# rohitsinghlab/SAME

Measured on AMD Instinct MI355X. Metric: cell-pairs/sec on 100k×100k cost build + edge-cross sweep; % HBM roofline, higher is better.
Workload: dtype f64

## Files before the change

### same_amd/csrc/delaunay_dev.hip

```cpp
#include "qhull_margin.h"
#include "window_internal.h"

namespace {

using namespace devmath;
using namespace win;
using scan::Pair;

constexpr int NB_CAP = 128;
constexpr int OWN_CAP = 32;
constexpr int SURV_CAP = 1024;
constexpr int SCAN_CELLS_CAP = 256;
constexpr double SIGN_MARGIN = 1e-12;
constexpr double SCREEN_SLACK = 1e-9;

enum { ST_STATUS = 0, ST_TRIS = 1, ST_WORDS = 8 };

struct Par {
    double x0, y0, cw, r2s, delta, w, sc_m;
    qm::Scale sc;
    double ox[8], oy[8];
    int nx, ny, ncell, n_oct;
};

struct Job {
    const double *xy;
    int64_t n, ncell_cap, cap_out;
    unsigned long long *st;
    unsigned long long *scan_cells, *scan_own;
    unsigned *cell_cnt, *cell_start, *slot, *own_cnt;
    int32_t *cell_of, *sorted, *own_tris, *out;
    Par *par;
};

struct Settings {
    double radius, cos_thr, guard;
};

__device__ __forceinline__ void refuse(const Job &j, unsigned bits) { atomicOr(&j.st[ST_STATUS], (unsigned long long)bits); }
__device__ __forceinline__ unsigned long long status_of(const Job &j) {
    return __hip_atomic_load(&j.st[ST_STATUS], __ATOMIC_RELAXED, __HIP_MEMORY_SCOPE_AGENT);
}
__device__ __forceinline__ int cell_x(const Par &p, double x) {
    const double f = std::floor((x - p.x0) / p.cw);
    return !(f >= 0.0) ? 0 : (f >= (double)p.nx ? p.nx - 1 : (int)f);
}
__device__ __forceinline__ int cell_y(const Par &p, double y) {
    const double f = std::floor((y - p.y0) / p.cw);
    return !(f >= 0.0) ? 0 : (f >= (double)p.ny ? p.ny - 1 : (int)f);
}

__device__ __forceinline__ double block_min(double v, double *sh) {
#pragma unroll
    for (int off = 32; off > 0; off >>= 1) v = fmin(v, __shfl_xor(v, off, 64));
    __syncthreads();
    if ((threadIdx.x & 63) == 0) sh[threadIdx.x >> 6] = v;
    __syncthreads();
    return fmin(fmin(sh[0], sh[1]), fmin(sh[2], sh[3]));
}
__device__ __forceinline__ void block_argmax(double &v, int64_t &i, double *shv, int64_t *shi) {
#pragma unroll
    for (int off = 32; off > 0; off >>= 1) {
        const double ov = __shfl_xor(v, off, 64);
        const int64_t oi = __shfl_xor(i, off, 64);
        if (ov > v || (ov == v && oi < i)) { v = ov; i = oi; }
    }
    __syncthreads();
    if ((threadIdx.x & 63) == 0) { shv[threadIdx.x >> 6] = v; shi[threadIdx.x >> 6] = i; }
    __syncthreads();
    v = shv[0];
    i = shi[0];
    for (int q = 1; q < 4; ++q)
        if (shv[q] > v || (shv[q] == v && shi[q] < i)) { v = shv[q]; i = shi[q]; }
}

__device__ __forceinline__ double oct_dir(int k, double x, double y) {
    switch (k) {
        case 0: return -y;
        case 1: return x - y;
        case 2: return x;
        case 3: return x + y;
        case 4: return y;
        case 5: return y - x;
        case 6: return -x;
        default: return -x - y;
    }
}

__global__ __launch_bounds__(256) void dd_setup_kernel(Batch<Job> b, Settings set) {
    const Job &j = b.w[blockIdx.y];
    __shared__ double shv[4];
    __shared__ int64_t shi[4];
    const int64_t n = j.n;
    double mnx = __builtin_inf(), mny = mnx, mxx = mnx, mxy = mnx, zmin = mnx, zmax = mnx, m = mnx;
    bool bad = false;
    double ov[8];
    int64_t oi[8];
    for (int k = 0; k < 8; ++k) { ov[k] = -__builtin_inf(); oi[k] = INT64_MAX; }
    for (int64_t i = threadIdx.x; i < n; i += blockDim.x) {
        const double x = j.xy[2 * i], y = j.xy[2 * i + 1];
        if (!(std::isfinite(x) && std::isfinite(y))) { bad = true; continue; }
        const double z = x * x + y * y;
        mnx = fmin(mnx, x); mxx = fmin(mxx, -x); mny = fmin(mny, y); mxy = fmin(mxy, -y);
        zmin = fmin(zmin, z); zmax = fmin(zmax, -z);
        m = fmin(m, -fmax(std::fabs(x), std::fabs(y)));
        for (int k = 0; k < 8; ++k) {
            const double v = oct_dir(k, x, y);
            if (v > ov[k] || (v == ov[k] && i < oi[k])) { ov[k] = v; oi[k] = i; }
        }
    }
    if (bad) refuse(j, SAME_DD_NONFINITE);
    mnx = block_min(mnx, shv); mxx = -block_min(mxx, shv); mny = block_min(mny, shv); mxy = -block_min(mxy, shv);
    zmin = block_min(zmin, shv); zmax = -block_min(zmax, shv); m = -block_min(m, shv);
    for (int k = 0; k < 8; ++k) block_argmax(ov[k], oi[k], shv, shi);
    if (threadIdx.x != 0) return;
    Par &p = *j.par;
    if (n < 3) { refuse(j, SAME_DD_FEW_POINTS); p.nx = p.ny = p.ncell = 1; p.n_oct = 0; p.x0 = p.y0 = 0.0; p.cw = 1.0; return; }
    p.sc = qm::scale(m, zmin, zmax);
    const double w = fmax(mxx - mnx, mxy - mny);
    p.w = w;
    p.sc_m = m;
    p.x0 = mnx;
    p.y0 = mny;
    p.r2s = (set.radius * (1.0 + SCREEN_SLACK)) * (set.radius * (1.0 + SCREEN_SLACK));
    double cw = set.radius * (1.0 + 1e-6);
    int64_t nx = 1, ny = 1;
    for (int it = 0; it < 64; ++it) {
        const double fx = std::floor((mxx - mnx) / cw) + 1.0, fy = std::floor((mxy - mny) / cw) + 1.0;
        if (fx * fy <= (double)j.ncell_cap) { nx = (int64_t)fx; ny = (int64_t)fy; break; }
        cw *= 2.0;
        nx = 0;
    }
    if (nx == 0 || !(cw > 0.0) || !std::isfinite(cw)) { refuse(j, SAME_DD_OVERFLOW); nx = ny = 1; }
    p.cw = cw;
    p.nx = (int)nx;
    p.ny = (int)ny;
    p.ncell = (int)(nx * ny);
    p.delta = 4.0 * set.guard * p.sc.allow + 64.0 * qm::EPS * (w + m);
    int c = 0;
    for (int k = 0; k < 8; ++k) {
        const int64_t i = oi[k];
        if (i < 0 || i >= n) continue;
        const double x = j.xy[2 * i], y = j.xy[2 * i + 1];
        if (c > 0 && x == p.ox[c - 1] && y == p.oy[c - 1]) continue;
        if (k == 7 && c > 0 && x == p.ox[0] && y == p.oy[0]) continue;
        p.ox[c] = x;
        p.oy[c] = y;
        ++c;
    }
    p.n_oct = c;
}

__global__ __launch_bounds__(256) void dd_count_kernel(Batch<Job> b) {
    const Job &j = b.w[blockIdx.y];
    const int64_t i = (int64_t)blockIdx.x * blockDim.x + threadIdx.x;
    if (i >= j.n || j.n < 3) return;
    const Par &p = *j.par;
    const int c = cell_y(p, j.xy[2 * i + 1]) * p.nx + cell_x(p, j.xy[2 * i]);
    j.cell_of[i] = c;
    j.slot[i] = atomicAdd(&j.cell_cnt[c], 1u);
}
__global__ __launch_bounds__(scan::NT) void dd_cell_scan_kernel(Batch<Job> b) {
    __shared__ scan::Shared sh;
    const Job &j = b.w[blockIdx.y];
    if (j.n < 3) return;
    const int64_t nc = j.par->ncell;
    const int nb = (int)scan::blocks_for(nc);
    if ((int)blockIdx.x >= nb) return;
    const unsigned *cnt = j.cell_cnt;
    auto val = [&](int64_t c) { return Pair{c < nc ? cnt[c] : 0u, 0u}; };
    Pair through;
    const Pair off = scan::exclusive(j.scan_cells, (int)blockIdx.x, val, sh, &through);
    const int64_t c = (int64_t)blockIdx.x * scan::NT + threadIdx.x;
    if (c < nc) j.cell_start[c] = off.a;
    if ((int)blockIdx.x == nb - 1 && threadIdx.x == 0) j.cell_start[nc] = through.a;
}
__global__ __launch_bounds__(256) void dd_scatter_kernel(Batch<Job> b) {
    const Job &j = b.w[blockIdx.y];
    const int64_t i = (int64_t)blockIdx.x * blockDim.x + threadIdx.x;
    if (i >= j.n || j.n < 3) return;
    const int64_t at = (int64_t)j.cell_start[j.cell_of[i]] + j.slot[i];
    if (at >= 0 && at < j.n) j.sorted[at] = (int32_t)i;
}
__global__ __launch_bounds__(256) void dd_cell_sort_kernel(Batch<Job> b) {
    const Job &j = b.w[blockIdx.y];
    const int64_t c = (int64_t)blockIdx.x * blockDim.x + threadIdx.x;
    if (j.n < 3 || c >= j.par->ncell) return;
    const int64_t lo = j.cell_start[c], hi = j.cell_start[c + 1];
    if (lo < 0 || hi > j.n) return;
    int32_t *s = j.sorted;
    for (int64_t a = lo + 1; a < hi; ++a) {
        const int32_t v = s[a];
        int64_t q = a - 1;
        while (q >= lo && s[q] > v) { s[q + 1] = s[q]; --q; }
        s[q + 1] = v;
    }
}

__device__ __forceinline__ double cross3(double ax, double ay, double bx, double by, double cx, double cy) {
    return (bx - ax) * (cy - ay) - (by - ay) * (cx - ax);
}

__global__ __launch_bounds__(256) void dd_hull_kernel(Batch<Job> b, Settings set) {
    const Job &j = b.w[blockIdx.y];
    if (j.n < 3 || status_of(j)) return;
    const Par &p = *j.par;
    __shared__ double ux[SURV_CAP], uy[SURV_CAP], sx[SURV_CAP], sy[SURV_CAP];
    __shared__ int32_t ui[SURV_CAP], si[SURV_CAP];
    __shared__ int hull[2 * SURV_CAP + 2];
    __shared__ int n_surv, n_hull, verdict;
    if (threadIdx.x == 0) { n_surv = 0; n_hull = 0; verdict = 0; }
    __syncthreads();
    const int n_oct = p.n_oct;
    for (int64_t i = threadIdx.x; i < j.n; i += blockDim.x) {
        const double x = j.xy[2 * i], y = j.xy[2 * i + 1];
        bool deep = n_oct >= 3;
        for (int k = 0; k < n_oct && deep; ++k) {
            const int k1 = k + 1 == n_oct ? 0 : k + 1;
            const double ex = p.ox[k1] - p.ox[k], ey = p.oy[k1] - p.oy[k];
            const double len = std::sqrt(ex * ex + ey * ey);
            deep = cross3(p.ox[k], p.oy[k], p.ox[k1], p.oy[k1], x, y) > p.delta * len + 16.0 * qm::EPS * (p.sc_m + p.w) * (len + 2.0 * p.w);
        }
        if (!deep) {
            const int at = atomicAdd(&n_surv, 1);
            if (at < SURV_CAP) { ux[at] = x; uy[at] = y; ui[at] = (int32_t)i; }
        }
    }
    __syncthreads();
    const int k = n_surv;
    if (k > SURV_CAP || k < 3) {
        if (threadIdx.x == 0) refuse(j, k > SURV_CAP ? SAME_DD_OVERFLOW : SAME_DD_IN_DOUBT);
        return;
    }
    for (int a = threadIdx.x; a < k; a += blockDim.x) {
        int r = 0;
        for (int c = 0; c < k; ++c)
            r += ux[c] < ux[a] || (ux[c] == ux[a] && (uy[c] < uy[a] || (uy[c] == uy[a] && ui[c] < ui[a])));
        sx[r] = ux[a]; sy[r] = uy[a]; si[r] = ui[a];
    }
    __syncthreads();
    if (threadIdx.x == 0) {
        int h = 0;
        for (int a = 0; a < k; ++a) {
            while (h >= 2 && cross3(sx[hull[h - 2]], sy[hull[h - 2]], sx[hull[h - 1]], sy[hull[h - 1]], sx[a], sy[a]) <= 0.0) --h;
            hull[h++] = a;
        }
        for (int a = k - 2, lo = h + 1; a >= 0; --a) {
            while (h >= lo && cross3(sx[hull[h - 2]], sy[hull[h - 2]], sx[hull[h - 1]], sy[hull[h - 1]], sx[a], sy[a]) <= 0.0) --h;
            hull[h++] = a;
        }
        n_hull = h - 1;
        if (n_hull < 3) verdict = 1;
    }
    __syncthreads();
    const int h = n_hull;
    if (!verdict) {
        for (int t = threadIdx.x; t < h; t += blockDim.x) {
            const int a = hull[(t + h - 1) % h], c = hull[t], d = hull[(t + 1) % h];
            const double area2 = std::fabs(cross3(sx[a], sy[a], sx[c], sy[c], sx[d], sy[d]));
            const double chord = std::sqrt((sx[d] - sx[a]) * (sx[d] - sx[a]) + (sy[d] - sy[a]) * (sy[d] - sy[a]));
            if (!(qm::plain_ratio(area2, chord, p.sc) > set.guard)) atomicOr(&verdict, 1);
        }
        for (int64_t q = threadIdx.x; q < (int64_t)k * h; q += blockDim.x) {
            const int s = (int)(q / h), e = (int)(q % h);
            const int a = hull[e], c = hull[(e + 1) % h];
            if (s == a || s == c) continue;
            const double area2 = std::fabs(cross3(sx[a], sy[a], sx[c], sy[c], sx[s], sy[s]));
            const double edge = std::sqrt((sx[c] - sx[a]) * (sx[c] - sx[a]) + (sy[c] - sy[a]) * (sy[c] - sy[a]));
            if (!(qm::plain_ratio(area2, edge, p.sc) > set.guard)) atomicOr(&verdict, 1);
        }
    }
    __syncthreads();
    if (threadIdx.x == 0 && verdict) refuse(j, SAME_DD_IN_DOUBT);
}

__device__ __forceinline__ double max_corner_cos(double2_t a, double2_t b, double2_t c) {
    const double c1 = corner_cos(b, a, c), c2 = corner_cos(a, b, c), c3 = corner_cos(a, c, b);
    return fmax(fmax(c1, c2), c3);
}

__global__ __launch_bounds__(256) void dd_candidate_kernel(Batch<Job> b, Settings set) {
    const Job &j = b.w[blockIdx.y];
    const int64_t pi = (int64_t)blockIdx.x * blockDim.x + threadIdx.x;
    if (pi >= j.n || j.n < 3 || status_of(j)) return;
    const Par &p = *j.par;
    const double *__restrict__ xy = j.xy;
    const int32_t *__restrict__ sorted = j.sorted;
    const unsigned *__restrict__ start = j.cell_start;
    const double2_t P = ld2(xy, pi);
    const int c0 = j.cell_of[pi], cx = c0 % p.nx, cy = c0 / p.nx;
    int32_t nb[NB_CAP];
    int k = 0;
    for (int yy = cy - 1; yy <= cy + 1; ++yy) {
        if (yy < 0 || yy >= p.ny) continue;
        for (int xx = cx - 1; xx <= cx + 1; ++xx) {
            if (xx < 0 || xx >= p.nx) continue;
            const int c = yy * p.nx + xx;
            for (unsigned q = start[c]; q < start[c + 1]; ++q) {
                const int32_t s = sorted[q];
                if (s <= pi) continue;
                const double2_t S = ld2(xy, s);
                const double dx = S.x - P.x, dy = S.y - P.y;
                if (dx * dx + dy * dy >= p.r2s) continue;
                if (k == NB_CAP) { refuse(j, SAME_DD_OVERFLOW); return; }
                nb[k++] = s;
            }
        }
    }
    for (int a = 1; a < k; ++a) {
        const int32_t v = nb[a];
        int q = a - 1;
        while (q >= 0 && nb[q] > v) { nb[q + 1] = nb[q]; --q; }
        nb[q + 1] = v;
    }
    int32_t *own = j.own_tris + pi * (int64_t)OWN_CAP * 3;
    unsigned count = 0;
    for (int a = 0; a < k; ++a) {
        const double2_t Q = ld2(xy, nb[a]);
        for (int bq = a + 1; bq < k; ++bq) {
            const double2_t R = ld2(xy, nb[bq]);
            const double qx = R.x - Q.x, qy = R.y - Q.y;
            if (qx * qx + qy * qy >= p.r2s) continue;
            if (!(max_corner_cos(P, Q, R) < set.cos_thr + SCREEN_SLACK)) continue;
            double2_t B = Q, C = R;
            int32_t ib = nb[a], ic = nb[bq];
            const double o = cross3(P.x, P.y, Q.x, Q.y, R.x, R.y);
            if (o < 0.0) { B = R; C = Q; ib = nb[bq]; ic = nb[a]; }
            const double dx = B.x - P.x, dy = B.y - P.y, ex = C.x - P.x, ey = C.y - P.y;
            const double bl = dx * dx + dy * dy, cl = ex * ex + ey * ey, d = dx * ey - dy * ex;
            if (!(d > 0.0)) { refuse(j, SAME_DD_IN_DOUBT); return; }
            const double ucx = (ey * bl - dy * cl) * 0.5 / d, ucy = (dx * cl - ex * bl) * 0.5 / d;
            const double ccx = P.x + ucx, ccy = P.y + ucy, rad = std::sqrt(ucx * ucx + ucy * ucy);
            const double jd = qm::judge(P.x, P.y, dx, dy, ex, ey, p.sc);
            const double reach = 2.0 * set.guard / (rad * d * jd) + 1e-9 * rad + 1e-12 * (std::fabs(ccx) + std::fabs(ccy));
            const int x_lo = cell_x(p, ccx - (rad + reach)), x_hi = cell_x(p, ccx + (rad + reach));
            const int y_lo = cell_y(p, ccy - (rad + reach)), y_hi = cell_y(p, ccy + (rad + reach));
            if (!(reach < 1e300) || (int64_t)(x_hi - x_lo + 1) * (y_hi - y_lo + 1) > SCAN_CELLS_CAP) { refuse(j, SAME_DD_OVERFLOW); return; }
            bool inside = false, doubt = false;
            for (int yy = y_lo; yy <= y_hi && !inside; ++yy) {
                for (int xx = x_lo; xx <= x_hi && !inside; ++xx) {
                    const int c = yy * p.nx + xx;
                    for (unsigned q = start[c]; q < start[c + 1]; ++q) {
                        const int32_t s = sorted[q];
                        if (s == pi || s == ib || s == ic) continue;
                        const double2_t S = ld2(xy, s);
                        const double ax_ = P.x - S.x, ay_ = P.y - S.y, bx_ = B.x - S.x, by_ = B.y - S.y, fx = C.x - S.x, fy = C.y - S.y;
                        const double ap = ax_ * ax_ + ay_ * ay_, bp = bx_ * bx_ + by_ * by_, cp = fx * fx + fy * fy;
                        const double det = ax_ * (by_ * cp - bp * fy) - ay_ * (bx_ * cp - bp * fx) + ap * (bx_ * fy - by_ * fx);
                        const double perm = (std::fabs(by_ * cp) + std::fabs(bp * fy)) * std::fabs(ax_) +
                                            (std::fabs(bx_ * cp) + std::fabs(bp * fx)) * std::fabs(ay_) +
                                            (std::fabs(bx_ * fy) + std::fabs(by_ * fx)) * ap;
                        if (!(std::fabs(det) > SIGN_MARGIN * perm) || !(std::fabs(det) * jd > set.guard)) {
                            doubt = true;
                            continue;
                        }
                        if (det > 0.0) { inside = true; break; }
                    }
                }
            }
            if (inside) continue;
            if (doubt) { refuse(j, SAME_DD_IN_DOUBT); return; }
            if (count == OWN_CAP) { refuse(j, SAME_DD_OVERFLOW); return; }
            own[3 * count] = (int32_t)pi;
            own[3 * count + 1] = ib;
            own[3 * count + 2] = ic;
            ++count;
        }
    }
    j.own_cnt[pi] = count;
}

__global__ __launch_bounds__(scan::NT) void dd_emit_kernel(Batch<Job> b) {
    __shared__ scan::Shared sh;
    const Job &j = b.w[blockIdx.y];
    if (j.n < 3) return;
    const int64_t n = j.n;
    const int nb = (int)scan::blocks_for(n);
    if ((int)blockIdx.x >= nb) return;
    const unsigned *cnt = j.own_cnt;
    auto val = [&](int64_t i) { return Pair{i < n ? cnt[i] : 0u, 0u}; };
    Pair through;
    const Pair off = scan::exclusive(j.scan_own, (int)blockIdx.x, val, sh, &through);
    const int64_t i = (int64_t)blockIdx.x * scan::NT + threadIdx.x;
    if (i < n) {
        const unsigned c = cnt[i];
        if (c > (unsigned)OWN_CAP || (int64_t)off.a + c > j.cap_out) {
            refuse(j, SAME_DD_OVERFLOW);
        } else {
            const int32_t *src = j.own_tris + i * (int64_t)OWN_CAP * 3;
            int32_t *dst = j.out + 3 * (int64_t)off.a;
            for (unsigned q = 0; q < 3 * c; ++q) dst[q] = src[q];
        }
    }
    if ((int)blockIdx.x == nb - 1 && threadIdx.x == 0) j.st[ST_TRIS] = through.a;
}

struct Layout {
    size_t o_st, o_scan_cells, o_cell_cnt, o_own_cnt, o_scan_own, zero_bytes, o_par, o_cell_start, o_cell_of, o_slot, o_sorted, o_own, total;
    int64_t ncell_cap;
};
Layout layout_for(int64_t n) {
    Layout l{};
    l.ncell_cap = 2 * n + 64;
    Carver cv;
    l.o_st = cv.take(ST_WORDS * 8);
    l.o_scan_cells = cv.take(scan::status_bytes(l.ncell_cap));
    l.o_cell_cnt = cv.take((size_t)l.ncell_cap * 4);
    l.o_own_cnt = cv.take((size_t)n * 4);
    l.o_scan_own = cv.take(scan::status_bytes(n));
    l.zero_bytes = cv.off;
    l.o_par = cv.take(sizeof(Par));
    l.o_cell_start = cv.take((size_t)(l.ncell_cap + 1) * 4);
    l.o_cell_of = cv.take((size_t)n * 4);
    l.o_slot = cv.take((size_t)n * 4);
    l.o_sorted = cv.take((size_t)n * 4);
    l.o_own = cv.take((size_t)n * OWN_CAP * 12);
    l.total = cv.off;
    return l;
}
Job job_on(char *base, const Layout &l, const double *xy, int64_t n, int32_t *out, int64_t cap_out) {
    Job j{};
    j.xy = xy;
    j.n = n;
    j.ncell_cap = l.ncell_cap;
    j.cap_out = cap_out;
    j.st = reinterpret_cast<unsigned long long *>(base + l.o_st);
    j.scan_cells = scan::arg(reinterpret_cast<unsigned long long *>(base + l.o_scan_cells));
    j.cell_cnt = reinterpret_cast<unsigned *>(base + l.o_cell_cnt);
    j.own_cnt = reinterpret_cast<unsigned *>(base + l.o_own_cnt);
    j.scan_own = scan::arg(reinterpret_cast<unsigned long long *>(base + l.o_scan_own));
    j.par = reinterpret_cast<Par *>(base + l.o_par);
    j.cell_start = reinterpret_cast<unsigned *>(base + l.o_cell_start);
    j.cell_of = reinterpret_cast<int32_t *>(base + l.o_cell_of);
    j.slot = reinterpret_cast<unsigned *>(base + l.o_slot);
    j.sorted = reinterpret_cast<int32_t *>(base + l.o_sorted);
    j.own_tris = reinterpret_cast<int32_t *>(base + l.o_own);
    j.out = out;
    return j;
}

int launch_group(same_ctx *ctx, const Job *jobs, int n_j, Settings set) {
    Batch<Job> b{};
    int64_t max_n = 0, max_cells = 0;
    for (int q = 0; q < n_j; ++q) {
        b.w[q] = jobs[q];
        max_n = std::max(max_n, jobs[q].n);
        max_cells = std::max(max_cells, jobs[q].ncell_cap);
    }
    const unsigned nw = (unsigned)n_j;
    SAME_LAUNCH(ctx, dd_setup_kernel, dim3(1, nw), dim3(256), 0, b, set);
    SAME_LAUNCH(ctx, dd_count_kernel, dim3(grid_for(max_n), nw), dim3(256), 0, b);
    SAME_LAUNCH(ctx, dd_cell_scan_kernel, dim3(scan::blocks_for(max_cells), nw), dim3(scan::NT), 0, b);
    SAME_LAUNCH(ctx, dd_scatter_kernel, dim3(grid_for(max_n), nw), dim3(256), 0, b);
    SAME_LAUNCH(ctx, dd_cell_sort_kernel, dim3(grid_for(max_cells), nw), dim3(256), 0, b);
    SAME_LAUNCH(ctx, dd_hull_kernel, dim3(1, nw), dim3(256), 0, b, set);
    SAME_LAUNCH(ctx, dd_candidate_kernel, dim3(grid_for(max_n), nw), dim3(256), 0, b, set);
    SAME_LAUNCH(ctx, dd_emit_kernel, dim3(scan::blocks_for(max_n), nw), dim3(scan::NT), 0, b);
    HIP_TRY(ctx, hipGetLastError());
    return SAME_OK;
}

bool settings_answerable(double radius, int angle_enabled, double cos_thr) {
    return radius > 0.0 && std::isfinite(radius) && angle_enabled && cos_thr == cos_thr && cos_thr < 0.9999;
}

}

extern "C" {

int same_window_delaunay(same_window *const *windows, int n_windows, double radius, int angle_enabled, double cos_thr, double guard,
                         int32_t *out_status, int64_t *out_n_tris) {
    same_ctx *ctx = nullptr;
    SAME_TRY(check_batch(windows, n_windows, &ctx));
    REQUIRE(ctx, out_status && out_n_tris && guard >= 0.0);
    for (int i = 0; i < n_windows; ++i) REQUIRE(ctx, windows[i]->staged == 2 && windows[i]->n_ua < ((int64_t)1 << 30));
    SAME_TRY(same_use(ctx));
    const bool ok = settings_answerable(radius, angle_enabled, cos_thr);
    const Settings set{radius, cos_thr, guard};
    std::vector<Job> jobs;
    std::vector<int> at((size_t)n_windows, -1);
    for (int i = 0; i < n_windows; ++i) {
        same_window *w = windows[i];
        w->dd_ok = 0;
        w->n_dd = 0;
        out_status[i] = !ok ? SAME_DD_NO_ANGLE : (w->n_ua < 3 ? SAME_DD_FEW_POINTS : 0);
        out_n_tris[i] = 0;
        if (out_status[i]) continue;
        const int64_t n = w->n_ua, cap_out = 2 * n;
        const Layout l = layout_for(n);
        SAME_TRY(ensure(ctx, w->dd_work, l.total));
        SAME_TRY(ensure(ctx, w->dd_tris, (size_t)cap_out * 12));
        at[(size_t)i] = (int)jobs.size();
        jobs.push_back(job_on(static_cast<char *>(w->dd_work.p), l, w->axy_c, n, static_cast<int32_t *>(w->dd_tris.p), cap_out));
        jobs.back().ncell_cap = l.ncell_cap;
    }
    if (jobs.empty()) return SAME_OK;
    int rc = SAME_OK;
    for (size_t g = 0; g < jobs.size() && rc == SAME_OK; g += SAME_LAUNCH_WINDOWS) {
        const int n_g = (int)std::min<size_t>(SAME_LAUNCH_WINDOWS, jobs.size() - g);
        ZeroArgs zr[SAME_LAUNCH_WINDOWS];
        for (int q = 0; q < n_g; ++q) {
            const Job &jb = jobs[g + (size_t)q];
            zr[q] = ZeroArgs{{jb.st, nullptr}, {layout_for(jb.n).zero_bytes, 0}};
        }
        rc = launch_zero(ctx, zr, n_g);
        if (rc == SAME_OK) rc = launch_group(ctx, jobs.data() + g, n_g, set);
    }
    unsigned long long *h = static_cast<unsigned long long *>(ctx->pinned);
    for (size_t q = 0; q < jobs.size() && rc == SAME_OK; ++q) {
        hipError_t e = hipMemcpyAsync(h + 2 * q, jobs[q].st, 16, hipMemcpyDeviceToHost, ctx->stream);
        ++ctx->stats[SAME_STAT_COPIES];
        if (e != hipSuccess) rc = same_fail(ctx, SAME_EIO, "device triangulation status", e);
    }
    if (rc != SAME_OK) {
        (void)hipStreamSynchronize(ctx->stream);
        return rc;
    }
    SAME_WAIT(ctx);
    for (int i = 0; i < n_windows; ++i) {
        if (at[(size_t)i] < 0) continue;
        const unsigned long long *s = h + 2 * at[(size_t)i];
        same_window *w = windows[i];
        out_status[i] = (int32_t)(s[0] & 0x7fffffffu);
        if (out_status[i] == 0) {
            w->n_dd = (int64_t)s[1];
            w->dd_ok = 1;
            out_n_tris[i] = w->n_dd;
        }
    }
    return SAME_OK;
}

int same_delaunay_filtered(same_ctx *ctx, const double *xy, int64_t n, double radius, int angle_enabled, double cos_thr, double guard,
                           int32_t *out_tris, int64_t cap, int64_t *out_n_tris, int32_t *out_status) {
    if (!ctx) return SAME_EINVAL;
    REQUIRE(ctx, (xy || n == 0) && out_n_tris && out_status && n >= 0 && n < ((int64_t)1 << 30) && cap >= 0 && (out_tris || cap == 0) &&
                     guard >= 0.0);
    *out_n_tris = 0;
    *out_status = !settings_answerable(radius, angle_enabled, cos_thr) ? SAME_DD_NO_ANGLE : (n < 3 ? SAME_DD_FEW_POINTS : 0);
    if (*out_status) return SAME_OK;
    SAME_TRY(same_use(ctx));
    const Layout l = layout_for(n);
    double *dxy = nullptr;
    char *work = nullptr;
    int32_t *dout = nullptr;
    SAME_TRY(up_as(ctx, SL_AXY, xy, (size_t)n * 2, &dxy));
    SAME_TRY(slot_as(ctx, SL_X, l.total, &work));
    SAME_TRY(slot_as(ctx, SL_TRIS, (size_t)(2 * n) * 3, &dout));
    Job jb = job_on(work, l, dxy, n, dout, 2 * n);
    SAME_FILL(ctx, work, 0, l.zero_bytes);
    SAME_TRY(launch_group(ctx, &jb, 1, Settings{radius, cos_thr, guard}));
    unsigned long long *h = static_cast<unsigned long long *>(ctx->pinned);
    SAME_COPY(ctx, h, jb.st, 16, hipMemcpyDeviceToHost);
    SAME_WAIT(ctx);
    *out_status = (int32_t)(h[0] & 0x7fffffffu);
    if (*out_status) return SAME_OK;
    const int64_t count = (int64_t)h[1];
    if (count > cap) return SAME_EINVAL;
    if (count) {
        SAME_COPY(ctx, out_tris, dout, (size_t)count * 12, hipMemcpyDeviceToHost);
        SAME_WAIT(ctx);
    }
    *out_n_tris = count;
    return SAME_OK;
}

}
```

Baseline: 634.9 billion.

## Restructure Delaunay candidate kernel into wave-per-point with shared-memory cell staging

Replaces the one-thread-per-point candidate kernel with a cell-strided grid where each block stages a 5x5 cell neighbourhood of points into LDS. Each wavefront handles one owner point and distributes neighbour gathering, candidate triangle setup and in-circle tests across its lanes using ballots. The aim is to remove divergent serial loops and repeated global gathers of point coordinates. It adds LDS pressure, extra syncs and counters, and a global fallback path when the stage overflows or a circle reaches beyond the staged area.

```diff
diff --git a/same_amd/csrc/delaunay_dev.hip b/same_amd/csrc/delaunay_dev.hip
--- a/same_amd/csrc/delaunay_dev.hip
+++ b/same_amd/csrc/delaunay_dev.hip
@@ -14,7 +14,7 @@
 constexpr double SIGN_MARGIN = 1e-12;
 constexpr double SCREEN_SLACK = 1e-9;
 
-enum { ST_STATUS = 0, ST_TRIS = 1, ST_WORDS = 8 };
+enum { ST_STATUS = 0, ST_TRIS = 1, ST_FAR = 2, ST_UNSTAGED = 3, ST_WORDS = 8 };
 
 struct Par {
     double x0, y0, cw, r2s, delta, w, sc_m;
@@ -278,96 +278,304 @@
     const double c1 = corner_cos(b, a, c), c2 = corner_cos(a, b, c), c3 = corner_cos(a, c, b);
     return fmax(fmax(c1, c2), c3);
 }
-
-__global__ __launch_bounds__(256) void dd_candidate_kernel(Batch<Job> b, Settings set) {
+__device__ __forceinline__ bool near_owner(const Par &p, double2_t P, double2_t S) {
+    const double dx = S.x - P.x, dy = S.y - P.y;
+    return !(dx * dx + dy * dy >= p.r2s);
+}
+__device__ __forceinline__ bool screened(const Par &p, const Settings &set, double2_t P, double2_t Q, double2_t R) {
+    const double qx = R.x - Q.x, qy = R.y - Q.y;
+    if (qx * qx + qy * qy >= p.r2s) return false;
+    return max_corner_cos(P, Q, R) < set.cos_thr + SCREEN_SLACK;
+}
+
+struct Cand {
+    double2_t B, C;
+    double jd;
+    int x_lo, x_hi, y_lo, y_hi;
+    bool swap;
+    unsigned bad;
+};
+__device__ __forceinline__ Cand setup_candidate(const Par &p, const Settings &set, double2_t P, double2_t Q, double2_t R) {
+    Cand t{};
+    const double o = cross3(P.x, P.y, Q.x, Q.y, R.x, R.y);
+    t.swap = o < 0.0;
+    t.B = t.swap ? R : Q;
+    t.C = t.swap ? Q : R;
+    const double dx = t.B.x - P.x, dy = t.B.y - P.y, ex = t.C.x - P.x, ey = t.C.y - P.y;
+    const double bl = dx * dx + dy * dy, cl = ex * ex + ey * ey, d = dx * ey - dy * ex;
+    if (!(d > 0.0)) { t.bad = SAME_DD_IN_DOUBT; return t; }
+    const double ucx = (ey * bl - dy * cl) * 0.5 / d, ucy = (dx * cl - ex * bl) * 0.5 / d;
+    const double ccx = P.x + ucx, ccy = P.y + ucy, rad = std::sqrt(ucx * ucx + ucy * ucy);
+    t.jd = qm::judge(P.x, P.y, dx, dy, ex, ey, p.sc);
+    const double reach = 2.0 * set.guard / (rad * d * t.jd) + 1e-9 * rad + 1e-12 * (std::fabs(ccx) + std::fabs(ccy));
+    t.x_lo = cell_x(p, ccx - (rad + reach));
+    t.x_hi = cell_x(p, ccx + (rad + reach));
+    t.y_lo = cell_y(p, ccy - (rad + reach));
+    t.y_hi = cell_y(p, ccy + (rad + reach));
+    if (!(reach < 1e300) || (int64_t)(t.x_hi - t.x_lo + 1) * (t.y_hi - t.y_lo + 1) > SCAN_CELLS_CAP) t.bad = SAME_DD_OVERFLOW;
+    return t;
+}
+__device__ __forceinline__ int in_circle(double2_t P, double2_t B, double2_t C, double2_t S, double jd, double guard) {
+    const double ax_ = P.x - S.x, ay_ = P.y - S.y, bx_ = B.x - S.x, by_ = B.y - S.y, fx = C.x - S.x, fy = C.y - S.y;
+    const double ap = ax_ * ax_ + ay_ * ay_, bp = bx_ * bx_ + by_ * by_, cp = fx * fx + fy * fy;
+    const double det = ax_ * (by_ * cp - bp * fy) - ay_ * (bx_ * cp - bp * fx) + ap * (bx_ * fy - by_ * fx);
+    const double perm = (std::fabs(by_ * cp) + std::fabs(bp * fy)) * std::fabs(ax_) +
+                        (std::fabs(bx_ * cp) + std::fabs(bp * fx)) * std::fabs(ay_) +
+                        (std::fabs(bx_ * fy) + std::fabs(by_ * fx)) * ap;
+    if (!(std::fabs(det) > SIGN_MARGIN * perm) || !(std::fabs(det) * jd > guard)) return -1;
+    return det > 0.0 ? 1 : 0;
+}
+
+constexpr int WAVE = 64;
+constexpr int CAND_WAVES = 4;
+constexpr int STAGE_H = 2;
+constexpr int STAGE_SIDE = 2 * STAGE_H + 1;
+constexpr int STAGE_CAP = 640;
+constexpr int CAND_BLOCKS = 2048;
+static_assert(NB_CAP <= 255, "neighbour positions are packed in 8 bits");
+
+struct WaveLists {
+    int32_t found[NB_CAP], found_at[NB_CAP];
+    int32_t nb[NB_CAP];
+    double nbx[NB_CAP], nby[NB_CAP];
+    int32_t c_ab[WAVE];
+    int32_t c_box[WAVE][4];
+    double c_jd[WAVE];
+};
+
+__device__ __forceinline__ void wave_sync() {
+    __builtin_amdgcn_fence(__ATOMIC_RELEASE, "wavefront");
+    __builtin_amdgcn_wave_barrier();
+    __builtin_amdgcn_fence(__ATOMIC_ACQUIRE, "wavefront");
+}
+__device__ __forceinline__ unsigned wave_status(const Job &j) {
+    return __builtin_amdgcn_readfirstlane((unsigned)(status_of(j) & 0x7fffffffu));
+}
+
+__global__ __launch_bounds__(CAND_WAVES * WAVE) void dd_candidate_kernel(Batch<Job> b, Settings set) {
     const Job &j = b.w[blockIdx.y];
-    const int64_t pi = (int64_t)blockIdx.x * blockDim.x + threadIdx.x;
-    if (pi >= j.n || j.n < 3 || status_of(j)) return;
+    if (j.n < 3) return;
     const Par &p = *j.par;
     const double *__restrict__ xy = j.xy;
     const int32_t *__restrict__ sorted = j.sorted;
     const unsigned *__restrict__ start = j.cell_start;
-    const double2_t P = ld2(xy, pi);
-    const int c0 = j.cell_of[pi], cx = c0 % p.nx, cy = c0 / p.nx;
-    int32_t nb[NB_CAP];
-    int k = 0;
-    for (int yy = cy - 1; yy <= cy + 1; ++yy) {
-        if (yy < 0 || yy >= p.ny) continue;
-        for (int xx = cx - 1; xx <= cx + 1; ++xx) {
-            if (xx < 0 || xx >= p.nx) continue;
-            const int c = yy * p.nx + xx;
-            for (unsigned q = start[c]; q < start[c + 1]; ++q) {
+    const int nx = p.nx, ny = p.ny;
+    const unsigned n = (unsigned)j.n;
+    __shared__ double sx[STAGE_CAP], sy[STAGE_CAP];
+    __shared__ int32_t si[STAGE_CAP];
+    __shared__ int row_at[STAGE_SIDE][STAGE_SIDE + 1];
+    __shared__ WaveLists lists[CAND_WAVES];
+    const int w = threadIdx.x / WAVE, lane = threadIdx.x % WAVE;
+    WaveLists &L = lists[w];
+    const unsigned long long below = (1ull << lane) - 1;
+
+    for (int c0 = blockIdx.x; c0 < p.ncell; c0 += gridDim.x) {
+        const unsigned lo0 = start[c0], hi0 = start[c0 + 1];
+        if (!(lo0 < hi0) || hi0 > n) continue;
+        const int cx = c0 % nx, cy = c0 / nx;
+        const int gx_lo = max(cx - STAGE_H, 0), gx_hi = min(cx + STAGE_H, nx - 1);
+        const int gy_lo = max(cy - STAGE_H, 0), gy_hi = min(cy + STAGE_H, ny - 1);
+        unsigned n_stage = 0;
+        bool sane = true;
+        for (int r = 0; r <= gy_hi - gy_lo; ++r) {
+            const int base = (gy_lo + r) * nx;
+            const unsigned f = start[base + gx_lo], e = start[base + gx_hi + 1];
+            sane = sane && f <= e && e <= n;
+            n_stage += e - f;
+        }
+        const bool staged = sane && n_stage <= (unsigned)STAGE_CAP;
+        __syncthreads();
+        if (staged) {
+            if (threadIdx.x < (gy_hi - gy_lo + 1) * (gx_hi - gx_lo + 2)) {
+                const int r = threadIdx.x / (gx_hi - gx_lo + 2), x = threadIdx.x % (gx_hi - gx_lo + 2);
+                unsigned at = 0;
+                for (int q = 0; q < r; ++q) at += start[(gy_lo + q) * nx + gx_hi + 1] - start[(gy_lo + q) * nx + gx_lo];
+                const int base = (gy_lo + r) * nx;
+                row_at[r][x] = (int)(at + start[base + gx_lo + x] - start[base + gx_lo]);
+            }
+            __syncthreads();
+            for (int k = threadIdx.x; k < (int)n_stage; k += blockDim.x) {
+                int r = 0;
+                while (k >= row_at[r][gx_hi - gx_lo + 1]) ++r;
+                const unsigned q = start[(gy_lo + r) * nx + gx_lo] + (unsigned)(k - row_at[r][0]);
                 const int32_t s = sorted[q];
-                if (s <= pi) continue;
                 const double2_t S = ld2(xy, s);
-                const double dx = S.x - P.x, dy = S.y - P.y;
-                if (dx * dx + dy * dy >= p.r2s) continue;
-                if (k == NB_CAP) { refuse(j, SAME_DD_OVERFLOW); return; }
-                nb[k++] = s;
+                si[k] = s;
+                sx[k] = S.x;
+                sy[k] = S.y;
             }
-        }
-    }
-    for (int a = 1; a < k; ++a) {
-        const int32_t v = nb[a];
-        int q = a - 1;
-        while (q >= 0 && nb[q] > v) { nb[q + 1] = nb[q]; --q; }
-        nb[q + 1] = v;
-    }
-    int32_t *own = j.own_tris + pi * (int64_t)OWN_CAP * 3;
-    unsigned count = 0;
-    for (int a = 0; a < k; ++a) {
-        const double2_t Q = ld2(xy, nb[a]);
-        for (int bq = a + 1; bq < k; ++bq) {
-            const double2_t R = ld2(xy, nb[bq]);
-            const double qx = R.x - Q.x, qy = R.y - Q.y;
-            if (qx * qx + qy * qy >= p.r2s) continue;
-            if (!(max_corner_cos(P, Q, R) < set.cos_thr + SCREEN_SLACK)) continue;
-            double2_t B = Q, C = R;
-            int32_t ib = nb[a], ic = nb[bq];
-            const double o = cross3(P.x, P.y, Q.x, Q.y, R.x, R.y);
-            if (o < 0.0) { B = R; C = Q; ib = nb[bq]; ic = nb[a]; }
-            const double dx = B.x - P.x, dy = B.y - P.y, ex = C.x - P.x, ey = C.y - P.y;
-            const double bl = dx * dx + dy * dy, cl = ex * ex + ey * ey, d = dx * ey - dy * ex;
-            if (!(d > 0.0)) { refuse(j, SAME_DD_IN_DOUBT); return; }
-            const double ucx = (ey * bl - dy * cl) * 0.5 / d, ucy = (dx * cl - ex * bl) * 0.5 / d;
-            const double ccx = P.x + ucx, ccy = P.y + ucy, rad = std::sqrt(ucx * ucx + ucy * ucy);
-            const double jd = qm::judge(P.x, P.y, dx, dy, ex, ey, p.sc);
-            const double reach = 2.0 * set.guard / (rad * d * jd) + 1e-9 * rad + 1e-12 * (std::fabs(ccx) + std::fabs(ccy));
-            const int x_lo = cell_x(p, ccx - (rad + reach)), x_hi = cell_x(p, ccx + (rad + reach));
-            const int y_lo = cell_y(p, ccy - (rad + reach)), y_hi = cell_y(p, ccy + (rad + reach));
-            if (!(reach < 1e300) || (int64_t)(x_hi - x_lo + 1) * (y_hi - y_lo + 1) > SCAN_CELLS_CAP) { refuse(j, SAME_DD_OVERFLOW); return; }
-            bool inside = false, doubt = false;
-            for (int yy = y_lo; yy <= y_hi && !inside; ++yy) {
-                for (int xx = x_lo; xx <= x_hi && !inside; ++xx) {
-                    const int c = yy * p.nx + xx;
-                    for (unsigned q = start[c]; q < start[c + 1]; ++q) {
-                        const int32_t s = sorted[q];
-                        if (s == pi || s == ib || s == ic) continue;
-                        const double2_t S = ld2(xy, s);
-                        const double ax_ = P.x - S.x, ay_ = P.y - S.y, bx_ = B.x - S.x, by_ = B.y - S.y, fx = C.x - S.x, fy = C.y - S.y;
-                        const double ap = ax_ * ax_ + ay_ * ay_, bp = bx_ * bx_ + by_ * by_, cp = fx * fx + fy * fy;
-                        const double det = ax_ * (by_ * cp - bp * fy) - ay_ * (bx_ * cp - bp * fx) + ap * (bx_ * fy - by_ * fx);
-                        const double perm = (std::fabs(by_ * cp) + std::fabs(bp * fy)) * std::fabs(ax_) +
-                                            (std::fabs(bx_ * cp) + std::fabs(bp * fx)) * std::fabs(ay_) +
-                                            (std::fabs(bx_ * fy) + std::fabs(by_ * fx)) * ap;
-                        if (!(std::fabs(det) > SIGN_MARGIN * perm) || !(std::fabs(det) * jd > set.guard)) {
-                            doubt = true;
-                            continue;
-                        }
-                        if (det > 0.0) { inside = true; break; }
+        } else if (threadIdx.x == 0) {
+            atomicAdd(&j.st[ST_UNSTAGED], 1ull);
+        }
+        __syncthreads();
+
+        auto span = [&](int yy, int xa, int xb, int &beg, int &end) {
+            if (staged) {
+                beg = row_at[yy - gy_lo][xa - gx_lo];
+                end = row_at[yy - gy_lo][xb - gx_lo + 1];
+            } else {
+                beg = (int)start[yy * nx + xa];
+                end = (int)min(start[yy * nx + xb + 1], n);
+            }
+        };
+        auto point = [&](int at, int32_t &s, double2_t &S) {
+            if (staged) {
+                s = si[at];
+                S = double2_t{sx[at], sy[at]};
+            } else {
+                s = sorted[at];
+                S = ld2(xy, s);
+            }
+        };
+
+        for (unsigned o = lo0 + w; o < hi0; o += CAND_WAVES) {
+            if (wave_status(j)) break;
+            const int32_t pi = sorted[o];
+            const double2_t P = ld2(xy, pi);
+            int k = 0;
+            for (int yy = max(cy - 1, 0); yy <= min(cy + 1, ny - 1); ++yy) {
+                int beg, end;
+                span(yy, max(cx - 1, 0), min(cx + 1, nx - 1), beg, end);
+                for (int q0 = beg; q0 < end; q0 += WAVE) {
+                    const int q = q0 + lane;
+                    bool hit = false;
+                    int32_t s = 0;
+                    if (q < end) {
+                        double2_t S;
+                        point(q, s, S);
+                        hit = s > pi && near_owner(p, P, S);
+                    }
+                    const unsigned long long m = __ballot(hit);
+                    const int at = k + __popcll(m & below);
+                    if (hit && at < NB_CAP) {
+                        L.found[at] = s;
+                        L.found_at[at] = q;
+                    }
+                    k += __popcll(m);
+                }
+            }
+            if (k > NB_CAP) {
+                if (lane == 0) refuse(j, SAME_DD_OVERFLOW);
+                break;
+            }
+            wave_sync();
+            for (int a = lane; a < k; a += WAVE) {
+                const int32_t v = L.found[a];
+                int r = 0;
+                for (int c = 0; c < k; ++c) r += L.found[c] < v;
+                int32_t s;
+                double2_t S;
+                point(L.found_at[a], s, S);
+                L.nb[r] = v;
+                L.nbx[r] = S.x;
+                L.nby[r] = S.y;
+            }
+            wave_sync();
+            int32_t *own = j.own_tris + (int64_t)pi * OWN_CAP * 3;
+            unsigned count = 0;
+            bool stop = false;
+            const int n_pair = k * (k - 1) / 2;
+            for (int t0 = 0; t0 < n_pair && !stop; t0 += WAVE) {
+                const int t = t0 + lane;
+                int a = 0, bq = 0;
+                bool keep = false;
+                unsigned bad = 0;
+                Cand cd{};
+                if (t < n_pair) {
+                    int rem = t;
+                    while (rem >= k - 1 - a) { rem -= k - 1 - a; ++a; }
+                    bq = a + 1 + rem;
+                    const double2_t Q{L.nbx[a], L.nby[a]}, R{L.nbx[bq], L.nby[bq]};
+                    if (screened(p, set, P, Q, R)) {
+                        cd = setup_candidate(p, set, P, Q, R);
+                        bad = cd.bad;
+                        keep = bad == 0;
                     }
                 }
+                if (__ballot(bad != 0)) {
+                    if (bad) refuse(j, bad);
+                    stop = true;
+                    break;
+                }
+                const unsigned long long mk = __ballot(keep);
+                if (keep) {
+                    const int at = __popcll(mk & below);
+                    L.c_ab[at] = a | bq << 8 | (cd.swap ? 1 << 16 : 0);
+                    L.c_box[at][0] = cd.x_lo;
+                    L.c_box[at][1] = cd.x_hi;
+                    L.c_box[at][2] = cd.y_lo;
+                    L.c_box[at][3] = cd.y_hi;
+                    L.c_jd[at] = cd.jd;
+                }
+                wave_sync();
+                const int n_c = __popcll(mk);
+                for (int c = 0; c < n_c; ++c) {
+                    const int ab = L.c_ab[c], ia = ab & 0xff, ib_ = (ab >> 8) & 0xff;
+                    const bool sw = (ab >> 16) != 0;
+                    const double2_t Q{L.nbx[ia], L.nby[ia]}, R{L.nbx[ib_], L.nby[ib_]};
+                    const double2_t B = sw ? R : Q, C = sw ? Q : R;
+                    const int32_t ib = sw ? L.nb[ib_] : L.nb[ia], ic = sw ? L.nb[ia] : L.nb[ib_];
+                    const int x_lo = L.c_box[c][0], x_hi = L.c_box[c][1], y_lo = L.c_box[c][2], y_hi = L.c_box[c][3];
+                    const double jd = L.c_jd[c];
+                    bool inside = false, doubt = false;
+                    auto test = [&](int at) {
+                        int32_t s;
+                        double2_t S;
+                        point(at, s, S);
+                        if (s == pi || s == ib || s == ic) return 0;
+                        return in_circle(P, B, C, S, jd, set.guard);
+                    };
+                    if (staged && x_lo >= gx_lo && x_hi <= gx_hi && y_lo >= gy_lo && y_hi <= gy_hi) {
+                        int total = 0;
+                        for (int yy = y_lo; yy <= y_hi; ++yy) total += row_at[yy - gy_lo][x_hi - gx_lo + 1] - row_at[yy - gy_lo][x_lo - gx_lo];
+                        for (int f0 = 0; f0 < total && !inside; f0 += WAVE) {
+                            int v = 0;
+                            if (f0 + lane < total) {
+                                int g = f0 + lane, yy = y_lo;
+                                for (;; ++yy) {
+                                    const int len = row_at[yy - gy_lo][x_hi - gx_lo + 1] - row_at[yy - gy_lo][x_lo - gx_lo];
+                                    if (g < len || yy == y_hi) break;
+                                    g -= len;
+                                }
+                                v = test(row_at[yy - gy_lo][x_lo - gx_lo] + g);
+                            }
+                            inside = __ballot(v > 0) != 0;
+                            doubt = doubt || __ballot(v < 0) != 0;
+                        }
+                    } else {
+                        if (lane == 0) atomicAdd(&j.st[ST_FAR], 1ull);
+                        for (int yy = y_lo; yy <= y_hi && !inside; ++yy) {
+                            const int beg = (int)start[yy * nx + x_lo], end = (int)min(start[yy * nx + x_hi + 1], n);
+                            for (int q0 = beg; q0 < end && !inside; q0 += WAVE) {
+                                int v = 0;
+                                if (q0 + lane < end) {
+                                    const int32_t s = sorted[q0 + lane];
+                                    if (s != pi && s != ib && s != ic) v = in_circle(P, B, C, ld2(xy, s), jd, set.guard);
+                                }
+                                inside = __ballot(v > 0) != 0;
+                                doubt = doubt || __ballot(v < 0) != 0;
+                            }
+                        }
+                    }
+                    if (inside) continue;
+                    if (doubt || count == OWN_CAP) {
+                        if (lane == 0) refuse(j, doubt ? SAME_DD_IN_DOUBT : SAME_DD_OVERFLOW);
+                        stop = true;
+                        break;
+                    }
+                    if (lane == 0) {
+                        own[3 * count] = pi;
+                        own[3 * count + 1] = ib;
+                        own[3 * count + 2] = ic;
+                    }
+                    ++count;
+                }
+                wave_sync();
             }
-            if (inside) continue;
-            if (doubt) { refuse(j, SAME_DD_IN_DOUBT); return; }
-            if (count == OWN_CAP) { refuse(j, SAME_DD_OVERFLOW); return; }
-            own[3 * count] = (int32_t)pi;
-            own[3 * count + 1] = ib;
-            own[3 * count + 2] = ic;
-            ++count;
-        }
-    }
-    j.own_cnt[pi] = count;
+            if (!stop && lane == 0) j.own_cnt[pi] = count;
+            wave_sync();
+        }
+    }
 }
 
 __global__ __launch_bounds__(scan::NT) void dd_emit_kernel(Batch<Job> b) {
@@ -454,7 +662,7 @@
     SAME_LAUNCH(ctx, dd_scatter_kernel, dim3(grid_for(max_n), nw), dim3(256), 0, b);
     SAME_LAUNCH(ctx, dd_cell_sort_kernel, dim3(grid_for(max_cells), nw), dim3(256), 0, b);
     SAME_LAUNCH(ctx, dd_hull_kernel, dim3(1, nw), dim3(256), 0, b, set);
-    SAME_LAUNCH(ctx, dd_candidate_kernel, dim3(grid_for(max_n), nw), dim3(256), 0, b, set);
+    SAME_LAUNCH(ctx, dd_candidate_kernel, dim3((unsigned)std::min<int64_t>(max_cells, CAND_BLOCKS), nw), dim3(CAND_WAVES * WAVE), 0, b, set);
     SAME_LAUNCH(ctx, dd_emit_kernel, dim3(scan::blocks_for(max_n), nw), dim3(scan::NT), 0, b);
     HIP_TRY(ctx, hipGetLastError());
     return SAME_OK;
```

New measurement: 635.1 billion, median of 6. No clear change (+0.0%).
